# j-wilson/GPflowPILCO

Measured on AMD Instinct MI355X. Metric: moment_matched_rollout_step_elements_per_sec, higher is better.
Workload: dtype f32; 1 GPU; C3 (BASELINE configs[2]): N=2000 d=8 D=8 H=40 fp32 drift moment-match step / closed rollout; recipe=baseline: BASELINE.md recipe: lengthscales log-U[0.3,3], GP-prior targets, fresh mu~U[0,1]^d / Sigm~; N=2000, d=8, D=8, H=40, B_per_gpu=256, B_total=256, B_this_rank=256, parallelism=dp1 over B (weak), recipe=baseline, steps_requested=418, diag_pairs=f64, offdiag_pairs=f32

## Files before the change

gpflowpilco_amd/_lib.py:

```python
from __future__ import annotations

import ctypes as C
import os

_HERE = os.path.dirname(os.path.abspath(__file__))
LIB_PATH = os.environ.get("GPFLOWPILCO_MM_LIB") or os.path.join(_HERE, "libgpflowpilco_mm.so")

MM_F32, MM_F64 = 0, 1
MM_DMAX = 32
MM_M_ALIGN = 128
MM_FULL_OUTPUT_COV = 1
MM_MODEL_UNCERTAINTY = 2
MM_FORCE_GENERIC = 4
MM_STAGE_DIAG = 8
MM_STAGE_OFFDIAG = 16
MM_STAGE_FINALIZE = 32
MM_FORCE_WORST_TIER = 64
MM_WORKSPACE_CURRENT = 128
MM_FORCE_ROUTE = 256
MM_NO_ROUTE = 512
MM_SUMS_CURRENT = 1024
MM_ISTAGE_OLD_SKIP_BOUND = 1 << 26
MM_ISTAGE_NO_BOUND_SKIP = 1 << 27

ERRORS = {
    -1: "MM_E_ARG: NULL pointer or non-positive size",
    -2: "MM_E_DIM: input dimension d exceeds MM_DMAX=32 or unsupported shape",
    -3: "MM_E_DTYPE: dtype must be MM_F32 or MM_F64",
    -4: "MM_E_WORKSPACE: workspace/packed buffer too small",
    -5: "MM_E_NO_C: model_uncertainty requested but the model was packed without C",
    -6: "MM_E_STATE: Euler update / closed rollout needs d == L and a full output covariance",
}

SIGNATURES = {
    "mm_abi_version": (C.c_int, []),
    "mm_packed_model_bytes": (C.c_size_t, [C.c_int] * 5),
    "mm_pack_model": (C.c_int, [C.c_void_p, C.c_size_t, C.c_int, C.c_int, C.c_int, C.c_int]
                      + [C.c_void_p] * 6 + [C.c_void_p]),
    "mm_pack_perm": (C.c_int, [C.c_void_p, C.c_size_t, C.c_int, C.c_int, C.c_int, C.c_int, C.c_void_p, C.c_void_p]),
    "mm_workspace_bytes": (C.c_size_t, [C.c_int] * 6),
    "mm_moment_match": (C.c_int, [C.c_void_p, C.c_size_t, C.c_int, C.c_int, C.c_int, C.c_int, C.c_int,
                                  C.c_void_p, C.c_void_p, C.c_int, C.c_double,
                                  C.c_void_p, C.c_void_p, C.c_void_p,
                                  C.c_void_p, C.c_size_t, C.c_void_p, C.c_void_p]),
    "mm_q_forward": (C.c_int, [C.c_void_p, C.c_size_t, C.c_int, C.c_int, C.c_int, C.c_int, C.c_int,
                               C.c_void_p, C.c_void_p, C.c_int,
                               C.c_void_p, C.c_void_p, C.c_void_p,
                               C.c_void_p, C.c_size_t, C.c_void_p, C.c_void_p]),
    "mm_Q_reduce_forward": (C.c_int, [C.c_void_p, C.c_size_t, C.c_int, C.c_int, C.c_int, C.c_int, C.c_int,
                                      C.c_int, C.c_double, C.c_void_p,
                                      C.c_void_p, C.c_size_t, C.c_void_p]),
    "mm_euler_update": (C.c_int, [C.c_int, C.c_int, C.c_int, C.c_double] + [C.c_void_p] * 8),
    "mm_expected_cost": (C.c_int, [C.c_int, C.c_int, C.c_int] + [C.c_void_p] * 6),
    "mm_offdiag_stats": (C.c_int, [C.c_void_p, C.c_size_t, C.c_int, C.c_int, C.c_int, C.c_int, C.c_int, C.c_int,
                                   C.c_void_p, C.c_size_t, C.c_void_p, C.c_void_p]),
    "mm_offdiag_worklist_len": (C.c_int, [C.c_int] * 6 + [C.c_void_p, C.c_size_t, C.c_void_p, C.c_void_p]),
    "mm_offdiag_skip_bounds": (C.c_int, [C.c_void_p, C.c_size_t, C.c_int, C.c_int, C.c_int, C.c_int, C.c_int, C.c_int,
                                         C.c_void_p, C.c_size_t, C.c_void_p, C.c_void_p, C.c_void_p]),
    "mm_route_estimates": (C.c_int, [C.c_void_p, C.c_size_t, C.c_int, C.c_int, C.c_int, C.c_int, C.c_int, C.c_int,
                                     C.c_void_p, C.c_size_t, C.c_void_p, C.c_void_p]),
    "mm_compose_workspace_bytes": (C.c_size_t, [C.c_int] * 4),
    "mm_compose_nd_workspace_bytes": (C.c_size_t, [C.c_int] * 5),
    "mm_compose_tape_bytes": (C.c_size_t, [C.c_int] * 6),
    "mm_compose_backward_workspace_bytes": (C.c_size_t, [C.c_int] * 4),
    "mm_policy_grad_bytes": (C.c_size_t, [C.c_int] * 3),
    "mm_compose_tape_bytes_nd": (C.c_size_t, [C.c_int] * 7),
    "mm_compose_backward_workspace_bytes_nd": (C.c_size_t, [C.c_int] * 6),
    "mm_policy_grad_bytes_nd": (C.c_size_t, [C.c_int] * 4),
    "mm_compose_nd_mixed_workspace_bytes": (C.c_size_t, [C.c_int] * 6),
    "mm_compose_tape_bytes_nd_mixed": (C.c_size_t, [C.c_int] * 8),
    "mm_compose_backward_workspace_bytes_nd_mixed": (C.c_size_t, [C.c_int] * 7),
    "mm_bwd_f32_supported": (C.c_int, [C.c_int]),
    "mm_backward_pair_aggregates_bytes": (C.c_size_t, [C.c_int] * 5),
    "mm_backward_pair_aggregates": (C.c_int, [C.c_void_p, C.c_size_t, C.c_int, C.c_int, C.c_int, C.c_int, C.c_int,
                                              C.c_void_p, C.c_void_p, C.c_int, C.c_void_p, C.c_size_t, C.c_void_p, C.c_size_t,
                                              C.c_void_p, C.c_size_t, C.c_void_p, C.c_void_p]),
    "mm_moment_match_backward_bytes": (C.c_size_t, [C.c_int] * 5),
    "mm_moment_match_backward_bytes_dtype": (C.c_size_t, [C.c_int] * 6),
    "mm_moment_match_backward": (C.c_int, [C.c_void_p, C.c_size_t, C.c_int, C.c_int, C.c_int, C.c_int, C.c_int,
                                           C.c_void_p, C.c_void_p, C.c_int,
                                           C.c_void_p, C.c_void_p, C.c_void_p,
                                           C.c_void_p, C.c_void_p, C.c_int,
                                           C.c_void_p, C.c_size_t, C.c_void_p, C.c_size_t,
                                           C.c_void_p, C.c_void_p]),
    "mm_moment_match_with_sums": (C.c_int, [C.c_void_p, C.c_size_t, C.c_int, C.c_int, C.c_int, C.c_int, C.c_int,
                                            C.c_void_p, C.c_void_p, C.c_int, C.c_double,
                                            C.c_void_p, C.c_void_p, C.c_void_p,
                                            C.c_void_p, C.c_size_t, C.c_void_p, C.c_size_t,
                                            C.c_void_p, C.c_void_p]),
# ... 133 lines not shown
```

gpflowpilco_amd/csrc/mm_common.h:

```cpp
#pragma once
#include <stddef.h>
#include <stdint.h>
#include "../../include/gpflowpilco_mm.h"

static inline size_t mm_align_up(size_t x, size_t a) { return (x + a - 1) / a * a; }
static inline int mm_round_up_int(int x, int a) { return (x + a - 1) / a * a; }
static inline size_t mm_elem_size(int dtype) { return dtype == MM_F64 ? 8 : 4; }

#define MM_ISTAGE_NO_ROUTE (1 << 20)
#define MM_ISTAGE_ROUTE (1 << 21)
#define MM_ISTAGE_NO_M56 (1 << 22)
#define MM_ISTAGE_OLD_OFFDIAG (1 << 23)
#define MM_ISTAGE_OLD_SPOLY56 (1 << 24)
#define MM_ISTAGE_OLD_DIAG_MAP (1 << 25)
#define MM_ISTAGE_OLD_SKIP_BOUND (1 << 26)
#define MM_ISTAGE_NO_BOUND_SKIP (1 << 27)

#define MM_PW_KERNELS 3

static inline int mm_num_pairs(int L, int flags) {
  return (flags & MM_FULL_OUTPUT_COV) ? L * (L + 1) / 2 : L;
}

static inline int mm_moment_deg(int d) { return d <= 8 ? 4 : 2; }
static inline long long mm_binom(int n, int k) {
  if (k < 0 || k > n) return 0;
  long long r = 1;
  for (int i = 1; i <= k; ++i) r = r * (n - k + i) / i;
  return r;
}
static inline int mm_mono_count(int n, int d) { return (int)mm_binom(d + n - 1, n); }
static inline int mm_mono_offset(int n, int d) { int o = 0; for (int m = 0; m < n; ++m) o += mm_mono_count(m, d); return o; }
static inline size_t mm_rank_table_entries(int d) {
  const int dk = d <= 8 ? 8 : 32, deg = mm_moment_deg(d);
  size_t n = 0, p = 1;
  for (int k = 1; k <= deg; ++k) { p *= dk; n += p; }
  return n;
}
static inline int mm_moment_cols(int d) { return mm_round_up_int(mm_mono_offset(mm_moment_deg(d) + 1, d), 16); }
static inline int mm_moment56_off5(int d) { return d <= 8 ? mm_round_up_int(mm_mono_count(4, d), 128) : 0; }
static inline int mm_moment56_off6(int d) { return d <= 8 ? mm_moment56_off5(d) + mm_round_up_int(mm_mono_count(5, d), 128) : 0; }
static inline int mm_moment56_cols(int d) { return d <= 8 ? mm_moment56_off6(d) + mm_round_up_int(mm_mono_count(6, d), 128) : 0; }
struct MMTab56 { int ins[6], last[6], n_i16, mult2, mult3, n_f32; size_t bytes; };
static inline MMTab56 mm_tab56(int d) {
  MMTab56 t;
  int o = 0;
  for (int m = 0; m < 6; ++m) { t.ins[m] = o; o += mm_mono_count(m, d) * 8; }
  for (int k = 0; k < 6; ++k) { t.last[k] = o; o += mm_mono_count(k, d); }
  t.n_i16 = mm_round_up_int(o, 8);
// ... 229 lines not shown
```

gpflowpilco_amd/csrc/mm_moments.hip:

```cpp
#include <hip/hip_runtime.h>
#include <math.h>
#include "mm_common.h"
#include "mm_mono.h"

typedef double f64x4m __attribute__((ext_vector_type(4)));

#define MM_GEMM_RB 64
#define MM_GEMM_NB 128
#define MM_GEMM_KB 32
#define MM_GEMM_AS 34
#define MM_GEMM_BS 144

__device__ __forceinline__ void mm_decode_pair_m(int p, int L, int& a, int& a2) {
  int r = p - L, i = 0;
  while (r >= L - 1 - i) { r -= L - 1 - i; ++i; }
  a = i; a2 = i + 1 + r;
}

__global__ __launch_bounds__(256) __attribute__((amdgpu_waves_per_eu(2, 2))) void k_wmom_gemm(const double* __restrict__ whR, const double* __restrict__ whC,
                                                      const double* __restrict__ Zm, int KMp, int L, int Mp, int B, int Po,
                                                      int nrb, int ncb, int nwork, int col_deg3,
                                                      const unsigned int* __restrict__ amaxc, const double* __restrict__ zmax2,
                                                      const int* __restrict__ gperm, double* __restrict__ mom) {
  const int orig = blockIdx.x;
// ... 285 lines not shown
      const int nsz = ksz >> LB;
      for (int idx = tid; idx < nsz; idx += 256) {
        double s = 0.0;
#pragma unroll
        for (int l = 0; l < DK; ++l) s = fma(cur[MM_PADI(l * nsz + idx)], dmu[l], s);
        oth[MM_PADI(idx)] = s;
      }
      __syncthreads();
      double* tsw = cur; cur = oth; oth = tsw;
      ksz = nsz;
      sign_binom = -sign_binom * (double)k / (double)(n - k + 1);
    }
    __syncthreads();
  }
  const double tot = mm_block_sum256m(total, red);
  if (tid == 0) s12[(size_t)b * Po + po] = tot + nh[0] * qh[0];
#undef MM_PADI
}

int mm_launch_wmom_full(const char* packed, const MMModelLayout& ml, char* ws, const MMWorkspaceLayout& wl,
                        int B, int L, int d, hipStream_t stream) {
  const int nrb = ((L - 1) * B + MM_GEMM_RB - 1) / MM_GEMM_RB, ncb = (ml.KMp + MM_GEMM_NB - 1) / MM_GEMM_NB;
  const long long nwork_ll = (long long)L * ncb * MM_MOM_SPLIT * nrb;
  if (nwork_ll <= 0 || nwork_ll > 0x7fffffffLL) return MM_E_DIM;
  hipLaunchKernelGGL(k_wmom_gemm, dim3((int)nwork_ll), dim3(256), 0, stream, (const double*)(ws + wl.whR),
                     (const double*)(ws + wl.whC), (const double*)(packed + ml.Zm), ml.KMp, L, wl.Mp, B, wl.Po, nrb, ncb,
                     (int)nwork_ll, 0x7fffffff , (const unsigned int*)nullptr, (const double*)(packed + ml.zmax2),
                     (const int*)nullptr, (double*)(ws + wl.mom));
  hipError_t e = hipGetLastError();
  return e == hipSuccess ? 0 : (int)e;
}

int mm_launch_moments56(const char* packed, const MMModelLayout& ml, char* ws, const MMWorkspaceLayout& wl,
                        int B, int L, int d, int allow, int old_spoly56, hipStream_t stream);

int mm_launch_moments(const char* packed, const MMModelLayout& ml, char* ws, const MMWorkspaceLayout& wl,
                      int B, int L, int d, const void* mu_f32, int flags, hipStream_t stream) {
  const double* Zm = (const double*)(packed + ml.Zm);
  double* mom = (double*)(ws + wl.mom);
  const int deg = mm_moment_deg(d) >= 4 ? 3 : mm_moment_deg(d);
  const int ncol_fwd = mm_mono_offset(deg + 1, d);
  const int nrb = ((L - 1) * B + MM_GEMM_RB - 1) / MM_GEMM_RB, ncb = (ncol_fwd + MM_GEMM_NB - 1) / MM_GEMM_NB;
  const long long nwork_ll = (long long)L * ncb * MM_MOM_SPLIT * nrb;
  if (nwork_ll <= 0 || nwork_ll > 0x7fffffffLL) return MM_E_DIM;
  const int nwork = (int)nwork_ll;
  const int allow = (flags & (MM_FORCE_WORST_TIER | MM_ISTAGE_NO_M56)) ? 0 : 1;
  const int col_deg3 = mm_mono_offset(3, d);
  const bool some = allow && mm_moment_deg(d) >= 4;
  if (some) {
    hipLaunchKernelGGL(k_wmom_perm, dim3(L), dim3(1024), 0, stream, (const unsigned int*)(ws + wl.amaxc),
                       (const double*)(packed + ml.zmax2), L, B, wl.Po, (int*)(ws + wl.gperm));
    hipError_t ep = hipGetLastError();
    if (ep != hipSuccess) return (int)ep;
  }
  hipLaunchKernelGGL(k_wmom_gemm, dim3(nwork), dim3(256), 0, stream, (const double*)(ws + wl.whR),
                     (const double*)(ws + wl.whC), Zm, ml.KMp, L, wl.Mp, B, wl.Po, nrb, ncb, nwork, col_deg3,
                     some ? (const unsigned int*)(ws + wl.amaxc) : (const unsigned int*)nullptr,
                     (const double*)(packed + ml.zmax2), some ? (const int*)(ws + wl.gperm) : (const int*)nullptr, mom);
  hipError_t e = hipGetLastError();
  if (e != hipSuccess) return (int)e;
  const int off1 = mm_mono_offset(1, d), off2 = mm_mono_offset(2, d), off3 = mm_mono_offset(3, d), off4 = mm_mono_offset(4, d);
#define MM_SPOLY(DK_, LB_)                                                                                                       \
  do {                                                                                                                          \
    const int dn_ = 1 << (LB_ * deg);                                                                                           \
    const int up_ = dn_ >> LB_;                                                                                                 \
    const size_t shm_ = (size_t)(dn_ + (dn_ >> 5) + up_ + (up_ >> 5) + 2 * ml.KMp + DK_ * DK_ + DK_ + 8) * sizeof(double);      \
    hipLaunchKernelGGL((k_spoly<DK_, LB_>), dim3(wl.Po, B), dim3(256), shm_, stream, (const double*)mom, ml.KMp,                \
                       (const double*)(ws + wl.pairmat), (const double*)(packed + ml.zbar), (const double*)(packed + ml.zmax2), \
                       (const unsigned int*)(ws + wl.amax), (const unsigned int*)(ws + wl.amaxc), (const float*)mu_f32, L, d, wl.P, deg, allow, off1, off2, off3, off4, \
                       (const short*)(packed + ml.rtab),                                                                        \
                       (double)MM_C6_C0, (double)MM_C6_C1, (double*)(ws + wl.s12));                                             \
  } while (0)
  if (d <= 8) MM_SPOLY(8, 3); else MM_SPOLY(32, 5);
#undef MM_SPOLY
  e = hipGetLastError();
  if (e != hipSuccess) return (int)e;
  if (flags & MM_ISTAGE_NO_M56) {
    if (mm_moment56_cols(d) <= 0 || wl.Po <= 0) return 0;
    const hipError_t em = hipMemsetAsync(ws + wl.s56, 0xFF, (size_t)B * wl.Po * sizeof(double), stream);
    if (em != hipSuccess) return (int)em;
    const hipError_t es = hipMemsetAsync(ws + wl.estS, 0, (size_t)B * wl.Po * sizeof(float), stream);
    return es == hipSuccess ? 0 : (int)es;
  }
  return mm_launch_moments56(packed, ml, ws, wl, B, L, d, some ? 1 : 0, (flags & MM_ISTAGE_OLD_SPOLY56) ? 1 : 0, stream);
}

__global__ void k_offdiag_stats(const unsigned int* __restrict__ amax, const double* __restrict__ zmax2,
                                const unsigned char* __restrict__ gflag, int ng, int L, int Po, int n,
                                int32_t* __restrict__ out) {
  const int idx = blockIdx.x * blockDim.x + threadIdx.x;
  bool c = false, in = false, part = false;
  int groups = 0;
  if (idx < n) {
    int a, a2;
    mm_decode_pair_m(L + idx % Po, L, a, a2);
    const float b2 = mm_collapse_bound2(amax[idx], zmax2[a2]);
    c = b2 <= MM_COLLAPSE_BOUND2;
    in = b2 <= MM_INSIDE_BOUND2;
    part = !c && mm_item_collapsed(amax[n + idx]);
    for (int g = 0; g < ng; ++g) groups += gflag[(size_t)idx * ng + g] ? 1 : 0;
  }
  const unsigned long long m = __ballot(c), mi = __ballot(in), mp = __ballot(part);
  if ((threadIdx.x & 63) == 0 && m) atomicAdd(out, (int)__popcll(m));
  if ((threadIdx.x & 63) == 0 && mi) atomicAdd(out + 2, (int)__popcll(mi));
  if ((threadIdx.x & 63) == 0 && mp) atomicAdd(out + 4, (int)__popcll(mp));
#pragma unroll
  for (int off = 32; off > 0; off >>= 1) groups += __shfl_down(groups, off, 64);
  if ((threadIdx.x & 63) == 0 && groups) atomicAdd(out + 5, groups);
  if (idx == 0) out[1] = n;
}

extern "C" int mm_offdiag_stats(const void* packed, size_t packed_bytes, int L, int M, int d, int dtype, int B, int flags,
                                const void* workspace, size_t workspace_bytes, int32_t* out, void* stream) {
  if (!packed || !workspace || !out || L <= 0 || M <= 0 || d <= 0 || d > MM_DMAX || B <= 0) return MM_E_ARG;
  const MMModelLayout ml = mm_model_layout(L, M, d, dtype, 1);
  const MMWorkspaceLayout wl = mm_workspace_layout(B, L, M, d, dtype, flags);
  if (packed_bytes < ml.Cm || workspace_bytes < wl.total) return MM_E_WORKSPACE;
// ... 16 lines not shown
```

gpflowpilco_amd/csrc/mm_moments6.hip:

```cpp
#include <hip/hip_runtime.h>
#include <math.h>
#include "mm_common.h"
#include "mm_mono.h"
#include "mm_f32_tile.h"
#include <atomic>
#include <type_traits>

__device__ __forceinline__ void mm6_decode_pair_o(int lp, int L, int& a, int& a2) {
  int r = lp, i = 0;
  while (r >= L - 1 - i) { r -= L - 1 - i; ++i; }
  a = i; a2 = i + 1 + r;
}

__global__ __launch_bounds__(256) void k_pack_zm56(char* packed, MMModelLayout lay, int L, int M, int d, int N56p,
                                                   const double* __restrict__ Z) {
  const int c = blockIdx.x, a = blockIdx.y, tid = threadIdx.x;
  const int n4 = mm_binom_i(d + 3, 4), n5 = mm_binom_i(d + 4, 5), n6 = mm_binom_i(d + 5, 6);
  const int off5 = ((n4 + 127) / 128) * 128;
  const int off6 = off5 + ((n5 + 127) / 128) * 128;
  const double* zbar = (const double*)(packed + lay.zbar) + (size_t)a * d;
  unsigned short* oh = (unsigned short*)(packed + lay.Zm56) + (((size_t)a * 2 + 0) * N56p + c) * lay.Mp;
  unsigned short* om = (unsigned short*)(packed + lay.Zm56) + (((size_t)a * 2 + 1) * N56p + c) * lay.Mp;
  int n = 0, k[6] = {0, 0, 0, 0, 0, 0};
  if (c < n4) { n = 4; mm_mono_unrank(c, 4, k); }
// ... 434 lines not shown
__global__ __launch_bounds__(256) void k_item_classes(const unsigned int* __restrict__ amaxc, const double* __restrict__ zmax2,
                                                      int L, int Po, int n, int allow, int* __restrict__ ilist,
                                                      double* __restrict__ s56, float* __restrict__ estS) {
  const int idx = blockIdx.x * 256 + threadIdx.x, lane = threadIdx.x & 63;
  int cls = 3;
  if (idx < n) {
    int a, a2;
    mm6_decode_pair_o(idx % Po, L, a, a2);
    const unsigned int ac = amaxc[idx];
    const float x2 = mm_collapse_bound2(ac, zmax2[a2]);
    cls = (!allow || !mm_item_collapsed(ac)) ? 3 : (x2 > MM_C6_X5_2 ? 0 : (x2 > MM_C6_X4_2 ? 1 : 2));
    if (cls == 3) { s56[idx] = 0.0; estS[idx] = 0.0f; }
  }
  const unsigned long long b01 = __ballot(cls == 0 || cls == 1), b2 = __ballot(cls == 2);
  int base01 = 0, base2 = 0;
  if (lane == 0) {
    if (b01) base01 = atomicAdd(ilist + 0, (int)__popcll(b01));
    if (b2) base2 = atomicAdd(ilist + 2, (int)__popcll(b2));
  }
  base01 = __shfl(base01, 0, 64); base2 = __shfl(base2, 0, 64);
  const unsigned long long below = (1ull << lane) - 1ull;
  if (cls == 0 || cls == 1) ilist[4 + base01 + __popcll(b01 & below)] = idx;
  if (cls == 2) ilist[4 + n - 1 - (base2 + __popcll(b2 & below))] = idx;
}

__device__ __forceinline__ float mm6_estS(float bound2, bool need5, bool need6, double r2, double c2) {
  const double X = sqrt((double)bound2), X3 = X * X * X;
  double amp = fmin(1.0, 64.0 * X3);
  if (!need6) amp += (double)MM_C6_C3 * X3 * X3 / 5.8e-10;
  if (!need5) amp += (double)MM_C6_C2 * X3 * X * X / 5.8e-10;
  return (float)fmin((double)MM_C6_SYS2 * (amp * amp) * r2 * c2, 3.0e38);
}

template <bool D8>
__global__ __launch_bounds__(MM6_THREADS) void k_spoly56(const float* __restrict__ mom56, int N56p, const double* __restrict__ pairmat,
                                                 const double* __restrict__ zmax2, const unsigned int* __restrict__ amaxc,
                                                 const unsigned char* __restrict__ gflag,
                                                 const double* __restrict__ whR, const double* __restrict__ whC,
                                                 const char* __restrict__ tab, MMTab56 tb, int L, int d_, int P, int Mp,
                                                 const int* __restrict__ ilist,
                                                 double* __restrict__ s56, float* __restrict__ estS) {
  extern __shared__ __align__(16) float sm6[];
  const int d = D8 ? 8 : d_;
  constexpr int NW = MM6_WAVES, NC = MM6_NC;
  const int tid = threadIdx.x;
  const int wave = __builtin_amdgcn_readfirstlane(tid >> 6), lane = tid & 63;
  const int Po = P - L;
  const int nitems = __builtin_amdgcn_readfirstlane(ilist[0]);
  for (int li = blockIdx.x; li < nitems; li += gridDim.x) {
  const size_t item = (size_t)__builtin_amdgcn_readfirstlane(ilist[4 + li]);
  const int b = (int)(item / Po), po = (int)(item - (size_t)b * Po);
  int a, a2;
  mm6_decode_pair_o(po, L, a, a2);
  const float bound2 = mm_collapse_bound2(amaxc[item], zmax2[a2]);
  int sy[7];
#pragma unroll
  for (int k = 0; k < 7; ++k) sy[k] = mm_binom_i(d + k - 1, k);
  const int n56 = sy[4] + sy[5] + sy[6];
  const int off5 = ((sy[4] + 127) / 128) * 128;
  const int off6 = off5 + ((sy[5] + 127) / 128) * 128;
  const bool need5 = bound2 > MM_C6_X4_2, need6 = bound2 > MM_C6_X5_2;
  const int xs = sy[3] + 1;
  float* nq = sm6;
  float* X = nq + 2 * n56;
  float* A = X + sy[3] * xs;
  float* Bf = A + sy[2] * sy[4];
  float* red = sm6 + ((2 * n56 + sy[3] * xs + sy[2] * sy[4] + sy[1] * sy[5] + 1) & ~1);
  for (int idx = tid; idx < 2 * n56; idx += MM6_THREADS) {
    const int side = idx >= n56, c = idx - side * n56;
    const int dg = c < sy[4] ? 4 : (c < sy[4] + sy[5] ? 5 : 6);
    const int col = dg == 4 ? c : (dg == 5 ? off5 + (c - sy[4]) : off6 + (c - sy[4] - sy[5]));
    float v = 0.0f;
    if (dg == 4 || (dg == 5 ? need5 : need6)) v = mom56[(item * 2 + side) * N56p + col];
    nq[idx] = v;
  }
  float* Gl = sm6 + ((2 * n56 + sy[3] * xs + sy[2] * sy[4] + sy[1] * sy[5] + 6 * MM6_WAVES + 2 + 3) & ~3);
  float* Bf4 = Gl + 128;
  float* X4 = Bf4 + sy[1] * sy[3];
  if (tid < 64) {
    const int i = tid >> 3, j = tid & 7;
    const double* pm = pairmat + ((size_t)b * P + (L + po)) * (d * d + 1);
    const float g = (i < d && j < d) ? (float)pm[i * d + j] : 0.0f;
    Gl[tid] = g;
    Gl[64 + j * 8 + i] = g;
  }
  double s2r = 0.0, s2c = 0.0;
  {
    const double* hr = whR + item * Mp;
    const double* hc = whC + item * Mp;
    const unsigned char* gf = gflag + item * (size_t)(Mp / MM_GROUP_ROWS);
    for (int m = tid; m < Mp; m += MM6_THREADS) {
      const double x = gf[m >> 6] ? hr[m] : 0.0, y = hc[m];
      s2r = fma(x, x, s2r); s2c = fma(y, y, s2c);
    }
  }
  __syncthreads();
  float G[64];
  auto load_G = [&](int transposed) __attribute__((always_inline)) {
#pragma unroll
    for (int q = 0; q < 16; ++q) {
      const float4 g4 = *reinterpret_cast<const float4*>(Gl + 64 * transposed + 4 * q);
      G[4 * q] = g4.x; G[4 * q + 1] = g4.y; G[4 * q + 2] = g4.z; G[4 * q + 3] = g4.w;
    }
  };
  const short* tabi = (const short*)tab;
  const float* mult2 = (const float*)(tab + (size_t)tb.n_i16 * 2) + tb.mult2;
  const float* mult3 = (const float*)(tab + (size_t)tb.n_i16 * 2) + tb.mult3;
  float acc5 = 0.0f, acc6 = 0.0f, dummy = 0.0f;
  if (need6) {
    const float* Q6 = nq + n56 + sy[4] + sy[5];
    const float* N6 = nq + sy[4] + sy[5];
    load_G(1);
    mm6_do<D8, 0, false, 0, NC, NW, 6, 0>(Q6, Bf, sy, tabi, tb, d, G, nullptr, 0, dummy, wave, lane);
    __syncthreads();
    mm6_do<D8, 1, false, 0, NC, NW, 5, 0>(Bf, A, sy, tabi, tb, d, G, nullptr, 0, dummy, wave, lane);
    __syncthreads();
    mm6_do<D8, 2, false, 1, NC, NW, 4, 121>(A, X, sy, tabi, tb, d, G, mult3, xs, dummy, wave, lane);
    __syncthreads();
    load_G(0);
    mm6_do<D8, 0, true, 0, NC, NW, 6, 0>(N6, Bf, sy, tabi, tb, d, G, nullptr, 0, dummy, wave, lane);
    __syncthreads();
    mm6_do<D8, 1, true, 0, NC, NW, 5, 0>(Bf, A, sy, tabi, tb, d, G, nullptr, 0, dummy, wave, lane);
    __syncthreads();
    mm6_do<D8, 2, true, 2, NC, NW, 4, 121>(A, X, sy, tabi, tb, d, G, nullptr, xs, acc6, wave, lane);
    __syncthreads();
  }
  float acc4 = 0.0f;
  {
    const float* Q5 = nq + n56 + sy[4];
    const float* N5 = nq + sy[4];
    const float* Q4 = nq + n56;
    const float* N4 = nq;
    const int xs4 = sy[2] + 1;
    load_G(1);
    if (need5) mm6_do<D8, 0, false, 0, NC, NW, 5, 0>(Q5, Bf, sy, tabi, tb, d, G, nullptr, 0, dummy, wave, lane);
    mm6_do<D8, 0, false, 0, NC, NW, 4, 0>(Q4, Bf4, sy, tabi, tb, d, G, nullptr, 0, dummy, wave, lane);
    __syncthreads();
    if (need5) mm6_do<D8, 1, false, 0, NC, NW, 4, 0>(Bf, A, sy, tabi, tb, d, G, nullptr, 0, dummy, wave, lane);
    mm6_do<D8, 1, false, 1, 1, NW, 3, 37>(Bf4, X4, sy, tabi, tb, d, G, mult2, xs4, dummy, wave, lane);
    __syncthreads();
    if (need5) {
      mm6_do<D8, 2, false, 1, 1, NW, 3, 121>(A, X, sy, tabi, tb, d, G, mult2, xs, dummy, wave, lane);
      __syncthreads();
    }
    load_G(0);
    if (need5) mm6_do<D8, 0, true, 0, NC, NW, 5, 0>(N5, Bf, sy, tabi, tb, d, G, nullptr, 0, dummy, wave, lane);
    mm6_do<D8, 0, true, 0, NC, NW, 4, 0>(N4, Bf4, sy, tabi, tb, d, G, nullptr, 0, dummy, wave, lane);
    __syncthreads();
    if (need5) mm6_do<D8, 1, true, 2, NC, NW, 4, 121>(Bf, X, sy, tabi, tb, d, G, nullptr, xs, acc5, wave, lane);
    mm6_do<D8, 1, true, 2, 1, NW, 3, 37>(Bf4, X4, sy, tabi, tb, d, G, nullptr, xs4, acc4, wave, lane);
  }
  double tot = (double)MM_C6_C1 * (double)acc4 + (double)MM_C6_C2 * (double)acc5 + (double)MM_C6_C3 * (double)acc6;
#pragma unroll
  for (int off = 32; off > 0; off >>= 1) {
    tot += __shfl_down(tot, off, 64); s2r += __shfl_down(s2r, off, 64); s2c += __shfl_down(s2c, off, 64);
  }
  double* redd = reinterpret_cast<double*>(red);
  if (lane == 0) { redd[wave * 3 + 0] = tot; redd[wave * 3 + 1] = s2r; redd[wave * 3 + 2] = s2c; }
  __syncthreads();
  if (tid == 0) {
    double t = 0.0, r2 = 0.0, c2 = 0.0;
    for (int w = 0; w < MM6_WAVES; ++w) { t += redd[w * 3]; r2 += redd[w * 3 + 1]; c2 += redd[w * 3 + 2]; }
    s56[item] = t;
    estS[item] = mm6_estS(bound2, need5, need6, r2, c2);
  }
  __syncthreads();
  }
}

template <bool D8>
__global__ __launch_bounds__(256) void k_spoly4(const float* __restrict__ mom56, int N56p, const double* __restrict__ pairmat,
                                                const double* __restrict__ zmax2, const unsigned int* __restrict__ amaxc,
                                                const unsigned char* __restrict__ gflag,
                                                const double* __restrict__ whR, const double* __restrict__ whC,
                                                const char* __restrict__ tab, MMTab56 tb, int L, int d_, int P, int Mp, int ntotal,
                                                const int* __restrict__ ilist,
                                                double* __restrict__ s56, float* __restrict__ estS) {
  extern __shared__ __align__(16) float sm4[];
  const int d = D8 ? 8 : d_;
  constexpr int NC0 = D8 ? 1 : MM6_NC;
  constexpr int NW = 4;
  const int tid = threadIdx.x;
  const int wave = __builtin_amdgcn_readfirstlane(tid >> 6), lane = tid & 63;
  const int Po = P - L;
  int sy[5];
#pragma unroll
  for (int k = 0; k < 5; ++k) sy[k] = mm_binom_i(d + k - 1, k);
  const int xs4 = sy[2] + 1;
  float* nq = sm4;
  float* Bf4 = nq + 2 * sy[4];
  float* X4 = Bf4 + sy[1] * sy[3];
  float* Gl = sm4 + ((2 * sy[4] + sy[1] * sy[3] + sy[2] * xs4 + 3) & ~3);
  double* redd = reinterpret_cast<double*>(Gl + 128);
  const short* tabi = (const short*)tab;
  const float* mult2 = (const float*)(tab + (size_t)tb.n_i16 * 2) + tb.mult2;
  const int nitems = __builtin_amdgcn_readfirstlane(ilist[2]);
  for (int li = blockIdx.x; li < nitems; li += gridDim.x) {
// ... 32 lines not shown
        G[4 * q] = g4.x; G[4 * q + 1] = g4.y; G[4 * q + 2] = g4.z; G[4 * q + 3] = g4.w;
      }
    };
    float acc4 = 0.0f, dummy = 0.0f;
    const float* Q4 = nq + sy[4];
    const float* N4 = nq;
    load_G(1);
    mm6_do<D8, 0, false, 0, NC0, NW, 4, 0>(Q4, Bf4, sy, tabi, tb, d, G, nullptr, 0, dummy, wave, lane);
    __syncthreads();
    mm6_do<D8, 1, false, 1, 1, NW, 3, 37>(Bf4, X4, sy, tabi, tb, d, G, mult2, xs4, dummy, wave, lane);
    __syncthreads();
    load_G(0);
    mm6_do<D8, 0, true, 0, NC0, NW, 4, 0>(N4, Bf4, sy, tabi, tb, d, G, nullptr, 0, dummy, wave, lane);
    __syncthreads();
    mm6_do<D8, 1, true, 2, 1, NW, 3, 37>(Bf4, X4, sy, tabi, tb, d, G, nullptr, xs4, acc4, wave, lane);
    double tot = (double)MM_C6_C1 * (double)acc4;
#pragma unroll
    for (int off = 32; off > 0; off >>= 1) {
      tot += __shfl_down(tot, off, 64); s2r += __shfl_down(s2r, off, 64); s2c += __shfl_down(s2c, off, 64);
    }
    if (lane == 0) { redd[wave * 3 + 0] = tot; redd[wave * 3 + 1] = s2r; redd[wave * 3 + 2] = s2c; }
    __syncthreads();
    if (tid == 0) {
      double t = 0.0, r2 = 0.0, c2 = 0.0;
      for (int w = 0; w < NW; ++w) { t += redd[w * 3]; r2 += redd[w * 3 + 1]; c2 += redd[w * 3 + 2]; }
      s56[item] = t;
      estS[item] = mm6_estS(bound2, false, false, r2, c2);
    }
    __syncthreads();
  }
}

int mm_launch_moments56(const char* packed, const MMModelLayout& ml, char* ws, const MMWorkspaceLayout& wl,
                        int B, int L, int d, int allow, int old_spoly56, hipStream_t stream) {
  const int N56p = mm_moment56_cols(d);
  if (N56p <= 0 || wl.Po <= 0) return 0;
  if (allow) {
    const int nrb = ((L - 1) * B + MM6_TB - 1) / MM6_TB, ncb = N56p / MM6_TB;
    const long long nwork_ll = (long long)L * ncb * nrb;
    if (nwork_ll <= 0 || nwork_ll > 0x7fffffffLL) return MM_E_DIM;
    if ((size_t)B * wl.Po * 4 * wl.Mp >= 0xffffffffull || (size_t)L * 2 * N56p * wl.Mp >= 0xffffffffull) return MM_E_DIM;
    const size_t shm = 2 * MM6_STAGE_BYTES + MM6_TB * sizeof(int);
    static std::atomic<unsigned long long> attr_done{0ull};
    int dev = 0;
    if (hipGetDevice(&dev) != hipSuccess) dev = 64;
    const unsigned long long bit = (dev >= 0 && dev < 64) ? (1ull << dev) : 0ull;
    if (!bit || !(attr_done.load() & bit)) {
      const hipError_t ea = hipFuncSetAttribute((const void*)k_wmom56_gemm, hipFuncAttributeMaxDynamicSharedMemorySize, (int)shm);
      if (ea != hipSuccess) return (int)ea;
      attr_done.fetch_or(bit);
    }
    hipLaunchKernelGGL(k_wmom56_gemm, dim3((int)nwork_ll), dim3(256), shm, stream, (const unsigned short*)(ws + wl.wsp),
                       (const unsigned short*)(packed + ml.Zm56), N56p, L, wl.Mp, B, wl.Po, nrb, ncb, (int)nwork_ll,
                       mm_moment56_off5(d) / MM6_TB, mm_moment56_off6(d) / MM6_TB,
                       (const int*)(ws + wl.gperm), (float*)(ws + wl.mom56));
    hipError_t e = hipGetLastError();
    if (e != hipSuccess) return (int)e;
  }
  const int nitem = B * wl.Po;
  int* ilist = (int*)(ws + wl.ilist);
  {
    const hipError_t em = hipMemsetAsync(ilist, 0, 16, stream);
    if (em != hipSuccess) return (int)em;
  }
  hipLaunchKernelGGL(k_item_classes, dim3((nitem + 255) / 256), dim3(256), 0, stream, (const unsigned int*)(ws + wl.amaxc),
                     (const double*)(packed + ml.zmax2), L, wl.Po, nitem, allow, ilist, (double*)(ws + wl.s56), (float*)(ws + wl.estS));
  {
    const hipError_t ec = hipGetLastError();
    if (ec != hipSuccess) return (int)ec;
  }
  if (!allow) return 0;
  int sy[7];
  for (int k = 0; k < 7; ++k) sy[k] = mm_mono_count(k, d);
  size_t nfl = (size_t)2 * (sy[4] + sy[5] + sy[6]) + (size_t)sy[3] * (sy[3] + 1) + (size_t)sy[2] * sy[4] + (size_t)sy[1] * sy[5] + 6 * MM6_WAVES + 128 + 16
               + (size_t)sy[1] * sy[3] + (size_t)sy[2] * (sy[2] + 1);
  nfl = (nfl + 1) & ~(size_t)1;
  const size_t shm = nfl * sizeof(float);
  static std::atomic<unsigned long long> attr2_done{0ull};
  static std::atomic<int> ncu_cached[64];
  int dev = 0;
  if (hipGetDevice(&dev) != hipSuccess) dev = 64;
  const unsigned long long bit2 = (dev >= 0 && dev < 64) ? (1ull << dev) : 0ull;
  int ncu = bit2 ? ncu_cached[dev].load() : 0;
  if (!bit2 || !(attr2_done.load() & bit2)) {
    hipError_t ea = hipFuncSetAttribute((const void*)k_spoly56<false>, hipFuncAttributeMaxDynamicSharedMemorySize, 160 * 1024);
    if (ea == hipSuccess) ea = hipFuncSetAttribute((const void*)k_spoly56<true>, hipFuncAttributeMaxDynamicSharedMemorySize, 160 * 1024);
    if (ea != hipSuccess) return (int)ea;
    int v = 0;
    if (hipDeviceGetAttribute(&v, hipDeviceAttributeMultiprocessorCount, dev < 64 ? dev : 0) != hipSuccess || v <= 0) v = 256;
    ncu = v;
    if (bit2) { ncu_cached[dev].store(v); attr2_done.fetch_or(bit2); }
  }
  if (ncu <= 0) ncu = 256;
  const int g56 = nitem < ncu ? nitem : ncu, g4 = nitem < 8 * ncu ? nitem : 8 * ncu;
  const bool d8 = d == 8 && !old_spoly56;
  hipLaunchKernelGGL((d8 ? k_spoly56<true> : k_spoly56<false>), dim3(g56), dim3(MM6_THREADS), shm, stream, (const float*)(ws + wl.mom56), N56p,
                     (const double*)(ws + wl.pairmat), (const double*)(packed + ml.zmax2), (const unsigned int*)(ws + wl.amaxc),
                     (const unsigned char*)(ws + wl.gflag), (const double*)(ws + wl.whR), (const double*)(ws + wl.whC),
                     packed + ml.tab56, mm_tab56(d), L, d, wl.P, wl.Mp, (const int*)ilist, (double*)(ws + wl.s56), (float*)(ws + wl.estS));
  {
    const hipError_t e5 = hipGetLastError();
    if (e5 != hipSuccess) return (int)e5;
  }
  const size_t shm4 = (size_t)(((2 * sy[4] + sy[1] * sy[3] + sy[2] * (sy[2] + 1) + 3) & ~3) + 128 + 2 * 3 * 4 + 8) * sizeof(float);
  hipLaunchKernelGGL((d8 ? k_spoly4<true> : k_spoly4<false>), dim3(g4), dim3(256), shm4, stream, (const float*)(ws + wl.mom56), N56p,
                     (const double*)(ws + wl.pairmat), (const double*)(packed + ml.zmax2), (const unsigned int*)(ws + wl.amaxc),
                     (const unsigned char*)(ws + wl.gflag), (const double*)(ws + wl.whR), (const double*)(ws + wl.whC),
                     packed + ml.tab56, mm_tab56(d), L, d, wl.P, wl.Mp, nitem, (const int*)ilist, (double*)(ws + wl.s56),
                     (float*)(ws + wl.estS));
  hipError_t e = hipGetLastError();
  return e == hipSuccess ? 0 : (int)e;
}
```

gpflowpilco_amd/ops.py:

```python
from __future__ import annotations

from dataclasses import dataclass, field
from typing import Dict, NamedTuple, Optional, Tuple

import torch

from . import _lib
from ._lib import (MM_F32, MM_F64, MM_FORCE_GENERIC, MM_FULL_OUTPUT_COV, MM_WORKSPACE_CURRENT, MM_SUMS_CURRENT,
                   MM_MODEL_UNCERTAINTY, check, lib)

_DTYPES = {torch.float32: MM_F32, torch.float64: MM_F64}


def _dtype_code(dtype: torch.dtype) -> int:
  try:
    return _DTYPES[dtype]
  except KeyError:
    raise TypeError(f"moment matching supports float32/float64 states, got {dtype}") from None


def _ptr(t: Optional[torch.Tensor]):
  return None if t is None else t.data_ptr()


# ... 183 lines not shown


def offdiag_row_groups(pm: PackedModel, B: int, flags: int):
  ws = pm.workspace(B, flags, peek=True)
  out = torch.zeros(6, dtype=torch.int32, device=pm.device)
  rc = lib().mm_offdiag_stats(pm.buf.data_ptr(), pm.nbytes, pm.L, pm.M, pm.d, _dtype_code(pm.dtype), B, flags,
                              ws.data_ptr(), ws.numel(), out.data_ptr(), _stream(pm.device))
  check(rc, "mm_offdiag_stats")
  o = out.tolist()
  Mp = (pm.M + _lib.MM_M_ALIGN - 1) // _lib.MM_M_ALIGN * _lib.MM_M_ALIGN
  return o[4], o[5], o[1] * (Mp // 64)


def offdiag_routed(pm: PackedModel, B: int, flags: int) -> int:
  if pm.dtype != torch.float32 or pm.L < 2 or not (flags & MM_FULL_OUTPUT_COV):
    return 0
  ws = pm.workspace(B, flags, peek=True)
  out = torch.zeros(6, dtype=torch.int32, device=pm.device)
  rc = lib().mm_offdiag_stats(pm.buf.data_ptr(), pm.nbytes, pm.L, pm.M, pm.d, _dtype_code(pm.dtype), B, flags,
                              ws.data_ptr(), ws.numel(), out.data_ptr(), _stream(pm.device))
  check(rc, "mm_offdiag_stats")
  return int(out[3])


def offdiag_worklist_len(pm: PackedModel, B: int, flags: int) -> int:
  if pm.dtype != torch.float32 or pm.L < 2 or not (flags & MM_FULL_OUTPUT_COV):
    return 0
  ws = pm.workspace(B, flags, peek=True)
  out = torch.zeros(1, dtype=torch.int32, device=pm.device)
  rc = lib().mm_offdiag_worklist_len(pm.L, pm.M, pm.d, _dtype_code(pm.dtype), B, flags, ws.data_ptr(), ws.numel(),
                                     out.data_ptr(), _stream(pm.device))
  check(rc, "mm_offdiag_worklist_len")
  return int(out[0])


def offdiag_skip_bounds(pm: PackedModel, B: int, flags: int):
  Mp = (pm.M + _lib.MM_M_ALIGN - 1) // _lib.MM_M_ALIGN * _lib.MM_M_ALIGN
  Po = pm.L * (pm.L - 1) // 2 if (flags & MM_FULL_OUTPUT_COV) else 0
  zt2s = torch.zeros(pm.L, Mp // 32, dtype=torch.float32, device=pm.device)
  gmax2s = torch.zeros(B, Po, Mp // 64, dtype=torch.float32, device=pm.device)
  ws = pm.workspace(B, flags, peek=True)
  rc = lib().mm_offdiag_skip_bounds(pm.buf.data_ptr(), pm.nbytes, pm.L, pm.M, pm.d, _dtype_code(pm.dtype), B, flags,
                                    ws.data_ptr(), ws.numel(), zt2s.data_ptr(), gmax2s.data_ptr(), _stream(pm.device))
  check(rc, "mm_offdiag_skip_bounds")
  return zt2s, gmax2s


def route_estimates(pm: PackedModel, B: int, flags: int) -> torch.Tensor:
  Po = pm.L * (pm.L - 1) // 2 if (flags & MM_FULL_OUTPUT_COV) else 0
  out = torch.zeros(B, Po, 2, dtype=torch.float64, device=pm.device)
  if Po:
    ws = pm.workspace(B, flags, peek=True)
    rc = lib().mm_route_estimates(pm.buf.data_ptr(), pm.nbytes, pm.L, pm.M, pm.d, _dtype_code(pm.dtype), B, flags,
                                  ws.data_ptr(), ws.numel(), out.data_ptr(), _stream(pm.device))
    check(rc, "mm_route_estimates")
  return out


def euler_update(mu, Sigma, f1, Sff, cross_pre, dt: float = 1.0):
  _require_device(mu, Sigma, f1, Sff, cross_pre)
  B, d = mu.shape
  if f1.shape != (B, d) or Sff.shape != (B, d, d) or cross_pre.shape != (B, d, d):
    raise ValueError("euler_update needs d == L and a full output covariance")
  args = [t.contiguous() for t in (mu, Sigma, f1, Sff, cross_pre)]
  mu_o, S_o = torch.empty_like(args[0]), torch.empty_like(args[1])
  rc = lib().mm_euler_update(B, d, _dtype_code(mu.dtype), float(dt), *[t.data_ptr() for t in args],
# ... 460 lines not shown
```

include/gpflowpilco_mm.h:

```cpp
#ifndef GPFLOWPILCO_MM_H
#define GPFLOWPILCO_MM_H

#include <stddef.h>
#include <stdint.h>

#ifdef __cplusplus
extern "C" {
#endif

#define MM_F32 0
#define MM_F64 1

#define MM_DMAX 32
#define MM_M_ALIGN 128

#define MM_FULL_OUTPUT_COV   1
#define MM_MODEL_UNCERTAINTY 2
#define MM_FORCE_GENERIC     4
#define MM_STAGE_DIAG        8
#define MM_STAGE_OFFDIAG    16
#define MM_STAGE_FINALIZE   32
#define MM_FORCE_WORST_TIER 64
#define MM_WORKSPACE_CURRENT 128
#define MM_FORCE_ROUTE 256
// ... 34 lines not shown
                    void* Sff,
                    void* cross_pre,
                    void* workspace, size_t workspace_bytes,
                    int32_t* status, void* stream);

int mm_q_forward(const void* packed, size_t packed_bytes, int L, int M, int d, int dtype, int B,
                 const void* mu, const void* Sigma, int flags,
                 void* f1, void* cross_pre, void* q_out,
                 void* workspace, size_t workspace_bytes, int32_t* status, void* stream);

int mm_Q_reduce_forward(const void* packed, size_t packed_bytes, int L, int M, int d, int dtype, int B,
                        int flags, double jitter, void* Sff,
                        void* workspace, size_t workspace_bytes, void* stream);

int mm_euler_update(int B, int d, int dtype, double dt,
                    const void* mu, const void* Sigma,
                    const void* f1, const void* Sff, const void* cross_pre,
                    void* mu_out, void* Sigma_out, void* stream);

int mm_rollout_closed(const void* packed, size_t packed_bytes, int L, int M, int d, int dtype, int B, int H,
                      double dt, int flags, double jitter,
                      void* mu, void* Sigma, void* traj_mu, void* traj_Sigma,
                      void* workspace, size_t workspace_bytes,
                      int32_t* status, void* stream);

int mm_expected_cost(int N, int d, int dtype, const void* mean, const void* cov,
                     const void* target, const void* precis, void* cost, void* stream);

int mm_offdiag_stats(const void* packed, size_t packed_bytes, int L, int M, int d, int dtype, int B, int flags,
                     const void* workspace, size_t workspace_bytes, int32_t* out, void* stream);

int mm_offdiag_worklist_len(int L, int M, int d, int dtype, int B, int flags, const void* workspace, size_t workspace_bytes,
                            int32_t* out, void* stream);

int mm_offdiag_skip_bounds(const void* packed, size_t packed_bytes, int L, int M, int d, int dtype, int B, int flags,
                           const void* workspace, size_t workspace_bytes, float* zt2s_out, float* gmax2s_out, void* stream);

int mm_route_estimates(const void* packed, size_t packed_bytes, int L, int M, int d, int dtype, int B, int flags,
                       const void* workspace, size_t workspace_bytes, double* out, void* stream);

size_t mm_compose_workspace_bytes(int B, int nx, int na, int dtype);
int mm_rollout_composed(const void* drift_packed, size_t drift_bytes, int drift_L, int drift_M, int drift_d,
                        const void* policy_packed, size_t policy_bytes, int policy_M, int policy_d,
                        int dtype, int B, int H, double dt, int nx, int na, const int32_t* active_dims,
                        double head_scale, double head_shift, const void* target, const void* precis,
                        void* mx, void* Sxx, void* cost, void* traj_mu, void* traj_Sigma,
                        void* ws_drift, size_t ws_drift_bytes, void* ws_policy, size_t ws_policy_bytes,
                        void* ws_compose, size_t ws_compose_bytes, int32_t* status, void* stream);

size_t mm_compose_nd_workspace_bytes(int B, int nx, int na, int nu, int dtype);
int mm_rollout_composed_nd(const void* drift_packed, size_t drift_bytes, int drift_L, int drift_M, int drift_d,
                           const void* policy_packed, size_t policy_bytes, int policy_M, int policy_d,
                           int dtype, int B, int H, double dt, int nx, int na, const int32_t* active_dims,
                           int nu, const double* head_scale, const double* head_shift,
                           const void* target, const void* precis,
                           void* mx, void* Sxx, void* cost, void* traj_mu, void* traj_Sigma,
                           void* ws_drift, size_t ws_drift_bytes, void* ws_policy, size_t ws_policy_bytes,
                           void* ws_compose, size_t ws_compose_bytes, int32_t* status, void* stream);

size_t mm_compose_tape_bytes(int B, int H, int nx, int na, int drift_M, int dtype);
int mm_rollout_composed_taped(const void* drift_packed, size_t drift_bytes, int drift_L, int drift_M, int drift_d,
                              const void* policy_packed, size_t policy_bytes, int policy_M, int policy_d,
                              int dtype, int B, int H, double dt, int nx, int na, const int32_t* active_dims,
                              double head_scale, double head_shift, const void* target, const void* precis,
                              void* mx, void* Sxx, void* cost, void* ws_drift, size_t ws_drift_bytes,
                              void* ws_policy, size_t ws_policy_bytes, void* tape, size_t tape_bytes,
// ... 259 lines not shown
```

Measured before the change: 45200 rollout step-elements/s (B*H per rollout second).

## Prefetch next work item's moments and norms in spare waves during spoly56 last phase

In the persistent k_spoly56 kernel, a subset of waves now fetches the next work item's mom56 columns (direct global-to-LDS loads), its G matrix and its whR/whC row norms while the other waves run the final contraction phase of the current item. The next iteration then skips its load prologue. The estS computation moves ahead of the compute and uses the prefetched norm reductions. This aims to hide global-memory latency between items, at the cost of more shared memory use, register pressure, and idling the prefetching waves during the last phase when d=8. A legacy flag and a debug worklist-length query are also added.

```diff
diff --git a/gpflowpilco_amd/_lib.py b/gpflowpilco_amd/_lib.py
--- a/gpflowpilco_amd/_lib.py
+++ b/gpflowpilco_amd/_lib.py
@@ -22,6 +22,7 @@
 MM_SUMS_CURRENT = 1024
 MM_ISTAGE_OLD_SKIP_BOUND = 1 << 26
 MM_ISTAGE_NO_BOUND_SKIP = 1 << 27
+MM_ISTAGE_OLD_SPOLY_LOAD = 1 << 28
 
 ERRORS = {
     -1: "MM_E_ARG: NULL pointer or non-positive size",
@@ -55,6 +56,7 @@
     "mm_offdiag_stats": (C.c_int, [C.c_void_p, C.c_size_t, C.c_int, C.c_int, C.c_int, C.c_int, C.c_int, C.c_int,
                                    C.c_void_p, C.c_size_t, C.c_void_p, C.c_void_p]),
     "mm_offdiag_worklist_len": (C.c_int, [C.c_int] * 6 + [C.c_void_p, C.c_size_t, C.c_void_p, C.c_void_p]),
+    "mm_moment56_worklist_len": (C.c_int, [C.c_int] * 6 + [C.c_void_p, C.c_size_t, C.c_void_p, C.c_void_p]),
     "mm_offdiag_skip_bounds": (C.c_int, [C.c_void_p, C.c_size_t, C.c_int, C.c_int, C.c_int, C.c_int, C.c_int, C.c_int,
                                          C.c_void_p, C.c_size_t, C.c_void_p, C.c_void_p, C.c_void_p]),
     "mm_route_estimates": (C.c_int, [C.c_void_p, C.c_size_t, C.c_int, C.c_int, C.c_int, C.c_int, C.c_int, C.c_int,
diff --git a/gpflowpilco_amd/csrc/mm_common.h b/gpflowpilco_amd/csrc/mm_common.h
--- a/gpflowpilco_amd/csrc/mm_common.h
+++ b/gpflowpilco_amd/csrc/mm_common.h
@@ -15,6 +15,7 @@
 #define MM_ISTAGE_OLD_DIAG_MAP (1 << 25)
 #define MM_ISTAGE_OLD_SKIP_BOUND (1 << 26)
 #define MM_ISTAGE_NO_BOUND_SKIP (1 << 27)
+#define MM_ISTAGE_OLD_SPOLY_LOAD (1 << 28)
 
 #define MM_PW_KERNELS 3
 
diff --git a/gpflowpilco_amd/csrc/mm_moments.hip b/gpflowpilco_amd/csrc/mm_moments.hip
--- a/gpflowpilco_amd/csrc/mm_moments.hip
+++ b/gpflowpilco_amd/csrc/mm_moments.hip
@@ -341,7 +341,7 @@
 }
 
 int mm_launch_moments56(const char* packed, const MMModelLayout& ml, char* ws, const MMWorkspaceLayout& wl,
-                        int B, int L, int d, int allow, int old_spoly56, hipStream_t stream);
+                        int B, int L, int d, int allow, int old_spoly56, int old_load, hipStream_t stream);
 
 int mm_launch_moments(const char* packed, const MMModelLayout& ml, char* ws, const MMWorkspaceLayout& wl,
                       int B, int L, int d, const void* mu_f32, int flags, hipStream_t stream) {
@@ -391,7 +391,8 @@
     const hipError_t es = hipMemsetAsync(ws + wl.estS, 0, (size_t)B * wl.Po * sizeof(float), stream);
     return es == hipSuccess ? 0 : (int)es;
   }
-  return mm_launch_moments56(packed, ml, ws, wl, B, L, d, some ? 1 : 0, (flags & MM_ISTAGE_OLD_SPOLY56) ? 1 : 0, stream);
+  return mm_launch_moments56(packed, ml, ws, wl, B, L, d, some ? 1 : 0, (flags & MM_ISTAGE_OLD_SPOLY56) ? 1 : 0,
+                             (flags & MM_ISTAGE_OLD_SPOLY_LOAD) ? 1 : 0, stream);
 }
 
 __global__ void k_offdiag_stats(const unsigned int* __restrict__ amax, const double* __restrict__ zmax2,
diff --git a/gpflowpilco_amd/csrc/mm_moments6.hip b/gpflowpilco_amd/csrc/mm_moments6.hip
--- a/gpflowpilco_amd/csrc/mm_moments6.hip
+++ b/gpflowpilco_amd/csrc/mm_moments6.hip
@@ -490,51 +490,61 @@
   return (float)fmin((double)MM_C6_SYS2 * (amp * amp) * r2 * c2, 3.0e38);
 }
 
+#define MM6_PFW 4
+#define MM6_PFU 3
 template <bool D8>
 __global__ __launch_bounds__(MM6_THREADS) void k_spoly56(const float* __restrict__ mom56, int N56p, const double* __restrict__ pairmat,
                                                  const double* __restrict__ zmax2, const unsigned int* __restrict__ amaxc,
                                                  const unsigned char* __restrict__ gflag,
                                                  const double* __restrict__ whR, const double* __restrict__ whC,
                                                  const char* __restrict__ tab, MMTab56 tb, int L, int d_, int P, int Mp,
-                                                 const int* __restrict__ ilist,
+                                                 const int* __restrict__ ilist, int prefetch,
                                                  double* __restrict__ s56, float* __restrict__ estS) {
   extern __shared__ __align__(16) float sm6[];
+  static_assert(MM6_WAVES % MM6_PFW == 0 && MM6_WAVES - MM6_PFW >= 8, "d = 8: the last phase's 8 units leave the prefetching waves idle");
   const int d = D8 ? 8 : d_;
   constexpr int NW = MM6_WAVES, NC = MM6_NC;
   const int tid = threadIdx.x;
   const int wave = __builtin_amdgcn_readfirstlane(tid >> 6), lane = tid & 63;
   const int Po = P - L;
   const int nitems = __builtin_amdgcn_readfirstlane(ilist[0]);
+  bool loaded = false;
   for (int li = blockIdx.x; li < nitems; li += gridDim.x) {
-  const size_t item = (size_t)__builtin_amdgcn_readfirstlane(ilist[4 + li]);
-  const int b = (int)(item / Po), po = (int)(item - (size_t)b * Po);
-  int a, a2;
-  mm6_decode_pair_o(po, L, a, a2);
-  const float bound2 = mm_collapse_bound2(amaxc[item], zmax2[a2]);
   int sy[7];
 #pragma unroll
   for (int k = 0; k < 7; ++k) sy[k] = mm_binom_i(d + k - 1, k);
   const int n56 = sy[4] + sy[5] + sy[6];
   const int off5 = ((sy[4] + 127) / 128) * 128;
   const int off6 = off5 + ((sy[5] + 127) / 128) * 128;
-  const bool need5 = bound2 > MM_C6_X4_2, need6 = bound2 > MM_C6_X5_2;
   const int xs = sy[3] + 1;
   float* nq = sm6;
   float* X = nq + 2 * n56;
   float* A = X + sy[3] * xs;
   float* Bf = A + sy[2] * sy[4];
   float* red = sm6 + ((2 * n56 + sy[3] * xs + sy[2] * sy[4] + sy[1] * sy[5] + 1) & ~1);
-  for (int idx = tid; idx < 2 * n56; idx += MM6_THREADS) {
+  double* redd = reinterpret_cast<double*>(red);
+  float* Gl = sm6 + ((2 * n56 + sy[3] * xs + sy[2] * sy[4] + sy[1] * sy[5] + 6 * MM6_WAVES + 2 + 3) & ~3);
+  float* Bf4 = Gl + 128;
+  float* X4 = Bf4 + sy[1] * sy[3];
+  auto nq_col = [&](int idx, bool need5, bool need6) __attribute__((always_inline)) {
     const int side = idx >= n56, c = idx - side * n56;
     const int dg = c < sy[4] ? 4 : (c < sy[4] + sy[5] ? 5 : 6);
     const int col = dg == 4 ? c : (dg == 5 ? off5 + (c - sy[4]) : off6 + (c - sy[4] - sy[5]));
+    return (dg == 4 || (dg == 5 ? need5 : need6)) ? side * N56p + col : -1;
+  };
+  const size_t item = (size_t)__builtin_amdgcn_readfirstlane(ilist[4 + li]);
+  const int b = (int)(item / Po), po = (int)(item - (size_t)b * Po);
+  int a, a2;
+  mm6_decode_pair_o(po, L, a, a2);
+  const float bound2 = mm_collapse_bound2(amaxc[item], zmax2[a2]);
+  const bool need5 = bound2 > MM_C6_X4_2, need6 = bound2 > MM_C6_X5_2;
+  if (!loaded) {
+  for (int idx = tid; idx < 2 * n56; idx += MM6_THREADS) {
+    const int col = nq_col(idx, need5, need6);
     float v = 0.0f;
-    if (dg == 4 || (dg == 5 ? need5 : need6)) v = mom56[(item * 2 + side) * N56p + col];
+    if (col >= 0) v = mom56[item * 2 * N56p + col];
     nq[idx] = v;
   }
-  float* Gl = sm6 + ((2 * n56 + sy[3] * xs + sy[2] * sy[4] + sy[1] * sy[5] + 6 * MM6_WAVES + 2 + 3) & ~3);
-  float* Bf4 = Gl + 128;
-  float* X4 = Bf4 + sy[1] * sy[3];
   if (tid < 64) {
     const int i = tid >> 3, j = tid & 7;
     const double* pm = pairmat + ((size_t)b * P + (L + po)) * (d * d + 1);
@@ -552,7 +562,16 @@
       s2r = fma(x, x, s2r); s2c = fma(y, y, s2c);
     }
   }
+#pragma unroll
+  for (int off = 32; off > 0; off >>= 1) { s2r += __shfl_down(s2r, off, 64); s2c += __shfl_down(s2c, off, 64); }
+  if (lane == 0) { redd[wave * 3 + 1] = s2r; redd[wave * 3 + 2] = s2c; }
   __syncthreads();
+  }
+  if (tid == 0) {
+    double r2 = 0.0, c2 = 0.0;
+    for (int w = 0; w < MM6_WAVES; ++w) { r2 += redd[w * 3 + 1]; c2 += redd[w * 3 + 2]; }
+    estS[item] = mm6_estS(bound2, need5, need6, r2, c2);
+  }
   float G[64];
   auto load_G = [&](int transposed) __attribute__((always_inline)) {
 #pragma unroll
@@ -605,22 +624,94 @@
     if (need5) mm6_do<D8, 0, true, 0, NC, NW, 5, 0>(N5, Bf, sy, tabi, tb, d, G, nullptr, 0, dummy, wave, lane);
     mm6_do<D8, 0, true, 0, NC, NW, 4, 0>(N4, Bf4, sy, tabi, tb, d, G, nullptr, 0, dummy, wave, lane);
     __syncthreads();
-    if (need5) mm6_do<D8, 1, true, 2, NC, NW, 4, 121>(Bf, X, sy, tabi, tb, d, G, nullptr, xs, acc5, wave, lane);
-    mm6_do<D8, 1, true, 2, 1, NW, 3, 37>(Bf4, X4, sy, tabi, tb, d, G, nullptr, xs4, acc4, wave, lane);
+    const int ln = li + (int)gridDim.x;
+    const bool fetch = prefetch && ln < nitems;
+    const bool fetcher = fetch && wave >= NW - MM6_PFW;
+    auto fetch_next = [&]() __attribute__((always_inline)) {
+      const int pw = wave - (NW - MM6_PFW);
+      int fl = lane;
+      asm volatile("" : "+v"(fl));
+      const size_t itn = (size_t)__builtin_amdgcn_readfirstlane(ilist[4 + ln]);
+      const int bn = (int)(itn / Po), pon = (int)(itn - (size_t)bn * Po);
+      const int gi = fl >> 3, gj = fl & 7;
+      const double gn = (pairmat + ((size_t)bn * P + (L + pon)) * (d * d + 1))[(gi < d ? gi : d - 1) * d + (gj < d ? gj : d - 1)];
+      constexpr int NV = MM6_WAVES / MM6_PFW;
+      const double* hr = whR + itn * Mp;
+      const double* hc = whC + itn * Mp;
+      const unsigned char* gf = gflag + itn * (size_t)(Mp / MM_GROUP_ROWS);
+      double xr[NV][MM6_PFU], xc[NV][MM6_PFU];
+      unsigned char xg[NV][MM6_PFU];
+#pragma unroll
+      for (int k = 0; k < NV; ++k)
+#pragma unroll
+        for (int u = 0; u < MM6_PFU; ++u) {
+          const int m = (pw + MM6_PFW * k) * 64 + fl + u * MM6_THREADS, mc = m < Mp ? m : Mp - 1;
+          xg[k][u] = gf[mc >> 6];
+          xr[k][u] = hr[mc];
+          xc[k][u] = hc[mc];
+        }
+      int an, a2n;
+      mm6_decode_pair_o(pon, L, an, a2n);
+      const float bound2n = mm_collapse_bound2(amaxc[itn], zmax2[a2n]);
+      const bool need5n = bound2n > MM_C6_X4_2, need6n = bound2n > MM_C6_X5_2;
+      const float* mq = mom56 + itn * 2 * N56p;
+      for (int base = pw * 64; base < 2 * n56; base += MM6_PFW * 64) {
+        const int idx = base + fl;
+        const int col = idx < 2 * n56 ? nq_col(idx, need5n, need6n) : 0;
+        if (idx < 2 * n56) {
+          if (col >= 0)
+            __builtin_amdgcn_global_load_lds((const __attribute__((address_space(1))) void*)(mq + col),
+                                             (__attribute__((address_space(3))) void*)(nq + base), 4, 0, 0);
+          else
+            nq[idx] = 0.0f;
+        }
+      }
+      if (pw == 0) {
+        const float g = (gi < d && gj < d) ? (float)gn : 0.0f;
+        Gl[fl] = g;
+        Gl[64 + gj * 8 + gi] = g;
+      }
+#pragma unroll
+      for (int k = 0; k < NV; ++k) {
+        const int w = pw + MM6_PFW * k, m0 = w * 64 + fl;
+        double s2r = 0.0, s2c = 0.0;
+#pragma unroll
+        for (int u = 0; u < MM6_PFU; ++u)
+          if (m0 + u * MM6_THREADS < Mp) {
+            const double x = xg[k][u] ? xr[k][u] : 0.0;
+            s2r = fma(x, x, s2r); s2c = fma(xc[k][u], xc[k][u], s2c);
+          }
+        for (int m = m0 + MM6_PFU * MM6_THREADS; m < Mp; m += MM6_THREADS) {
+          const double x = gf[m >> 6] ? hr[m] : 0.0, y = hc[m];
+          s2r = fma(x, x, s2r); s2c = fma(y, y, s2c);
+        }
+#pragma unroll
+        for (int off = 32; off > 0; off >>= 1) { s2r += __shfl_down(s2r, off, 64); s2c += __shfl_down(s2c, off, 64); }
+        if (fl == 0) { redd[w * 3 + 1] = s2r; redd[w * 3 + 2] = s2c; }
+      }
+      asm volatile("s_waitcnt vmcnt(0)" ::: "memory");
+    };
+    auto last_phase = [&]() __attribute__((always_inline)) {
+      if (need5) mm6_do<D8, 1, true, 2, NC, NW, 4, 121>(Bf, X, sy, tabi, tb, d, G, nullptr, xs, acc5, wave, lane);
+      mm6_do<D8, 1, true, 2, 1, NW, 3, 37>(Bf4, X4, sy, tabi, tb, d, G, nullptr, xs4, acc4, wave, lane);
+    };
+    if constexpr (D8) {
+      if (fetcher) fetch_next(); else last_phase();
+    } else {
+      if (fetcher) fetch_next();
+      last_phase();
+    }
+    loaded = fetch;
   }
   double tot = (double)MM_C6_C1 * (double)acc4 + (double)MM_C6_C2 * (double)acc5 + (double)MM_C6_C3 * (double)acc6;
 #pragma unroll
-  for (int off = 32; off > 0; off >>= 1) {
-    tot += __shfl_down(tot, off, 64); s2r += __shfl_down(s2r, off, 64); s2c += __shfl_down(s2c, off, 64);
-  }
-  double* redd = reinterpret_cast<double*>(red);
-  if (lane == 0) { redd[wave * 3 + 0] = tot; redd[wave * 3 + 1] = s2r; redd[wave * 3 + 2] = s2c; }
+  for (int off = 32; off > 0; off >>= 1) tot += __shfl_down(tot, off, 64);
+  if (lane == 0) redd[wave * 3 + 0] = tot;
   __syncthreads();
   if (tid == 0) {
-    double t = 0.0, r2 = 0.0, c2 = 0.0;
-    for (int w = 0; w < MM6_WAVES; ++w) { t += redd[w * 3]; r2 += redd[w * 3 + 1]; c2 += redd[w * 3 + 2]; }
+    double t = 0.0;
+    for (int w = 0; w < MM6_WAVES; ++w) t += redd[w * 3];
     s56[item] = t;
-    estS[item] = mm6_estS(bound2, need5, need6, r2, c2);
   }
   __syncthreads();
   }
@@ -719,7 +810,7 @@
 }
 
 int mm_launch_moments56(const char* packed, const MMModelLayout& ml, char* ws, const MMWorkspaceLayout& wl,
-                        int B, int L, int d, int allow, int old_spoly56, hipStream_t stream) {
+                        int B, int L, int d, int allow, int old_spoly56, int old_load, hipStream_t stream) {
   const int N56p = mm_moment56_cols(d);
   if (N56p <= 0 || wl.Po <= 0) return 0;
   if (allow) {
@@ -784,7 +875,8 @@
   hipLaunchKernelGGL((d8 ? k_spoly56<true> : k_spoly56<false>), dim3(g56), dim3(MM6_THREADS), shm, stream, (const float*)(ws + wl.mom56), N56p,
                      (const double*)(ws + wl.pairmat), (const double*)(packed + ml.zmax2), (const unsigned int*)(ws + wl.amaxc),
                      (const unsigned char*)(ws + wl.gflag), (const double*)(ws + wl.whR), (const double*)(ws + wl.whC),
-                     packed + ml.tab56, mm_tab56(d), L, d, wl.P, wl.Mp, (const int*)ilist, (double*)(ws + wl.s56), (float*)(ws + wl.estS));
+                     packed + ml.tab56, mm_tab56(d), L, d, wl.P, wl.Mp, (const int*)ilist, old_load ? 0 : 1, (double*)(ws + wl.s56),
+                     (float*)(ws + wl.estS));
   {
     const hipError_t e5 = hipGetLastError();
     if (e5 != hipSuccess) return (int)e5;
@@ -798,3 +890,18 @@
   hipError_t e = hipGetLastError();
   return e == hipSuccess ? 0 : (int)e;
 }
+
+extern "C" int mm_moment56_worklist_len(int L, int M, int d, int dtype, int B, int flags, const void* workspace, size_t workspace_bytes,
+                                        int32_t* out, void* stream) {
+  if (!workspace || !out || L <= 0 || M <= 0 || d <= 0 || d > MM_DMAX || B <= 0) return MM_E_ARG;
+  const MMWorkspaceLayout wl = mm_workspace_layout(B, L, M, d, dtype, flags);
+  if (workspace_bytes < wl.total) return MM_E_WORKSPACE;
+  hipStream_t s = (hipStream_t)stream;
+  hipError_t e = hipMemsetAsync(out, 0, 2 * sizeof(int32_t), s);
+  if (e != hipSuccess) return (int)e;
+  if (dtype != MM_F32 || wl.Po == 0 || d > 8) return 0;
+  const int32_t* ilist = (const int32_t*)((const char*)workspace + wl.ilist);
+  e = hipMemcpyAsync(out, ilist, sizeof(int32_t), hipMemcpyDeviceToDevice, s);
+  if (e == hipSuccess) e = hipMemcpyAsync(out + 1, ilist + 2, sizeof(int32_t), hipMemcpyDeviceToDevice, s);
+  return e == hipSuccess ? 0 : (int)e;
+}
diff --git a/gpflowpilco_amd/ops.py b/gpflowpilco_amd/ops.py
--- a/gpflowpilco_amd/ops.py
+++ b/gpflowpilco_amd/ops.py
@@ -239,6 +239,16 @@
                                      out.data_ptr(), _stream(pm.device))
   check(rc, "mm_offdiag_worklist_len")
   return int(out[0])
+
+
+def moment56_worklist_len(pm: PackedModel, B: int, flags: int):
+  ws = pm.workspace(B, flags, peek=True)
+  out = torch.zeros(2, dtype=torch.int32, device=pm.device)
+  rc = lib().mm_moment56_worklist_len(pm.L, pm.M, pm.d, _dtype_code(pm.dtype), B, flags, ws.data_ptr(), ws.numel(),
+                                      out.data_ptr(), _stream(pm.device))
+  check(rc, "mm_moment56_worklist_len")
+  n56, n4 = out.tolist()
+  return n56, n4
 
 
 def offdiag_skip_bounds(pm: PackedModel, B: int, flags: int):
diff --git a/include/gpflowpilco_mm.h b/include/gpflowpilco_mm.h
--- a/include/gpflowpilco_mm.h
+++ b/include/gpflowpilco_mm.h
@@ -90,6 +90,9 @@
 
 int mm_offdiag_worklist_len(int L, int M, int d, int dtype, int B, int flags, const void* workspace, size_t workspace_bytes,
                             int32_t* out, void* stream);
+
+int mm_moment56_worklist_len(int L, int M, int d, int dtype, int B, int flags, const void* workspace, size_t workspace_bytes,
+                             int32_t* out, void* stream);
 
 int mm_offdiag_skip_bounds(const void* packed, size_t packed_bytes, int L, int M, int d, int dtype, int B, int flags,
                            const void* workspace, size_t workspace_bytes, float* zt2s_out, float* gmax2s_out, void* stream);
```

Result: faster. 45810 rollout step-elements/s (B*H per rollout second), median of 6 (+1.4%).
